# neeek2303/EMOPortraits

Measured on AMD Instinct MI355X. Metric: reenactment frames/sec @512x512, 1-src->N-driver, higher is better.
Workload: dtype f32

## Files before the change

### emoportraits_amd/csrc/conv_igemm_f16x2_p1.h

```cpp
#pragma once
#include "conv_igemm_bf16x3.h"

template <int TR, int TW>
struct ConvCfgP {
  static constexpr int BM = 64, BP = 256, TM = 2, TP = 2, WGP = 4, KC = 32, NPL = 2;
  static constexpr int NQ = TW / 4;
  static constexpr int SUB = ((TR * NQ + 4 + 11) / 16) * 16 + 4;
  static constexpr int CHS = 4 * SUB;
  static constexpr int NG = 4;
  static constexpr int PPL = NG * CHS;
  static constexpr int PBUF = NPL * PPL;
  static constexpr int OFF_P = 0;
  static constexpr int WTILE = NPL * 2 * 2 * BM;
  static constexpr int WTILE_BYTES = WTILE * 16;
  static constexpr int WSTAGE = 2 * WTILE;
  static constexpr int OFF_W = 2 * PBUF;
  static constexpr int OFF_SCT = OFF_W + 2 * WSTAGE;
  static constexpr int SCT = 1024;
  static constexpr int EPI_ROWF = 68;
  static constexpr int EPI_WAVE = 32 * EPI_ROWF;
  static constexpr int OFF_BIAS_F = OFF_SCT * 4 + 2 * SCT;
  static constexpr int OFF_STAT_F = OFF_BIAS_F + BM;
  static constexpr int OFF_BIAS2_F = OFF_STAT_F + 2 * WGP * BM;
  static constexpr int OFF_STAT2_F = OFF_BIAS2_F + BM;
  static constexpr int LDS_BYTES = (OFF_STAT2_F + 2 * WGP * BM) * 4;
  static_assert(TR * TW == BP && TR * NQ == 64, "256 positions = 64 quads: one per lane of the staging wave");
  static_assert(WTILE_BYTES == 8 * 1024, "8 DMA pieces per channel tile and stage");
  static_assert(PBUF * 4 >= WGP * EPI_WAVE, "the epilogue transposes through one patch buffer");
  static_assert(LDS_BYTES <= 160 * 1024, "LDS");
};

template <int TR, int TW>
__global__ __launch_bounds__(256) __attribute__((amdgpu_waves_per_eu(1, 1)))
void conv_igemm_bf16x3_p1_kernel(const ConvArgs a) {
  using Cfg = ConvCfgP<TR, TW>;
  using opx8 = halfx8;
  constexpr int SPLIT = 2, NPL = 2, NPROD = 3;
  constexpr int BM = Cfg::BM, TM = Cfg::TM, TP = Cfg::TP, WGP = Cfg::WGP, KC = Cfg::KC;
  constexpr int NQ = Cfg::NQ, SUB = Cfg::SUB, CHS = Cfg::CHS, PPL = Cfg::PPL, PBUF = Cfg::PBUF;

  extern __shared__ __attribute__((aligned(16))) float smem[];

  EMO_SPLIT_THREAD_IDS()
  const int wp = wave;
  const int p0 = wp * TP * 32;
  float sat_m = 0.0f;

  const int HW = a.H * a.W;
  const long DHW = (long)a.D * HW;
  const bool has_affine = a.scale != nullptr;
  const int epi_mode = __builtin_amdgcn_readfirstlane(a.res == nullptr ? 0 : (a.res_ups ? 2 : 1));
  const float in_scale = a.in_scale;
  constexpr float CLAMP_HI = 65504.0f;
  const float clamp_lo = a.relu_in ? 0.0f : -CLAMP_HI;
  const int nst = a.n_cchunks;
  const int nptiles = a.tiles_x * a.tiles_y * a.tiles_z;
  const int n_cot_all = (a.Cout + BM - 1) / BM;

  const int q_r = lane / NQ, q_c = lane - q_r * NQ;
  int q_slb[4];
#pragma unroll
  for (int i = 0; i < 4; ++i) q_slb[i] = (wave * CHS + i * SUB + lane) * 16;

  floatx16 acc_lo[2][TM][TP], acc_hi[2][TM][TP];

  EMO_SPLIT_ITEM_WALK()
  int it_cotile = 0, it_n = 0, it_ptile = 0, it_x0 = 0, it_y0 = 0, it_z0 = 0;
  unsigned lq_off = 0;
  int lq_z0 = 0;
#define EMO_P1_WPTR(c_, k_) (reinterpret_cast<const char*>(a.wpk) + (long)((c_) * nst + (k_)) * Cfg::WTILE_BYTES)
#define EMO_P1_CURSOR_OF(P_, off_) { off_ = (unsigned)((P_##y0 + q_r) * a.W + P_##x0 + 4 * q_c) * 4u; }

  const int a_off = (half * BM + l32) * 16;
  int b_off[TP];
#pragma unroll
  for (int j = 0; j < TP; ++j) {
    const int p = p0 + j * 32 + l32;
    const int col = p % TW, row = p / TW;
    b_off[j] = (half * CHS + (col & 3) * SUB + row * NQ + (col >> 2)) * 16;
  }
  EMO_SPLIT_LDS_VIEWS()
  opx8 fa_[2][NPL][TM];
  opx8 fb_[2][NPL][TP];
#define EMO_P1_LOAD_A(set_, wb_, h_, ks_)                                                             \
  { _Pragma("unroll") for (int pl = 0; pl < NPL; ++pl) _Pragma("unroll") for (int i = 0; i < TM; ++i) \
      fa_[set_][pl][i] = *reinterpret_cast<const opx8*>(lds_c + a_off + (Cfg::OFF_W + (wb_) * Cfg::WSTAGE + (h_) * Cfg::WTILE + ((pl * 2 + (ks_)) * 2) * BM + i * 32) * 16); }
#define EMO_P1_LOAD_B(pb_, ks_)                                                                       \
  { _Pragma("unroll") for (int pl = 0; pl < NPL; ++pl) _Pragma("unroll") for (int j = 0; j < TP; ++j) \
      fb_[ks_][pl][j] = *reinterpret_cast<const opx8*>(lds_c + b_off[j] + (Cfg::OFF_P + (pb_) * PBUF + pl * PPL + (ks_) * 2 * CHS) * 16); }

  EMO_SPLIT_LDS_TABLES_ADDR()

  floatx4 qv[2][8];
  float q_lo[2], q_hi[2];
  int q_tix[2];
  floatx4 t_sc[2], t_sh[2];
  opx8 cv_h, cv_m;
  emo_intx4 xrs = emo_raw_buffer(a.x);
  EMO_SPLIT_USOFF(8, 0, DHW, 1u)

  int ld_stage;
  unsigned q_vo;
#define EMO_P1_ISSUE_BEGIN(b_)                                                                        \
  EMO_SPLIT_ISSUE_BEGIN([b_], q_vo, ld_stage * KC + wave * 8, cv_, ((unsigned)cs_ * (unsigned)DHW + (unsigned)(lq_z0 * HW)) * 4u)
#define EMO_P1_ISSUE_LOADS(b_) EMO_SPLIT_ISSUE_LOADS(qv[b_], q_vo, 0, 8)
#define EMO_P1_TABLES(b_) EMO_SPLIT_TABLE2(q_tix[b_], t_sc, t_sh)
#define EMO_P1_TOUCH_QUAD(b_) EMO_SPLIT_TOUCH(qv[b_], 8)
#define EMO_P1_CONV_HALF(b_, pb_, i_, hf_)                                                            \
  {                                                                                                   \
    EMO_SPLIT_AFFINE4(t_, qv[b_], 4 * (hf_), i_, t_sc[hf_], t_sh[hf_])                                \
    EMO_SPLIT_RANGE4(t_)                                                                              \
    EMO_SPLIT_F16X2_4(t_, q_lo[b_], q_hi[b_], cv_h, cv_m, 4 * (hf_))                                  \
    if ((hf_) == 1) {                                                                                 \
      char* d_ = lds_w + q_slb[i_] + (Cfg::OFF_P + (pb_) * PBUF) * 16;                                \
      EMO_SPLIT_STORE_PLANES(opx8, d_, cv_h, cv_m)                                                    \
    }                                                                                                 \
  }
#define EMO_P1_DMA_PIECE(ptr0_, ptr1_, wb_, k_)                                                       \
  {                                                                                                   \
    const int j_ = wave + 4 * ((k_) & 1);                                                             \
    emo_dma16_pinned_s((((k_) >> 1) ? (ptr1_) : (ptr0_)) + j_ * 1024, lane16,                         \
                       smem_lds + (unsigned)((Cfg::OFF_W + (wb_) * Cfg::WSTAGE + ((k_) >> 1) * Cfg::WTILE) * 16 + j_ * 1024)); \
  }

  constexpr int PA3[3] = {1, 0, 0}, PB3[3] = {0, 1, 0};
  constexpr int NTE = Cfg::SCT / 256;
  float te_sc[NTE], te_sh[NTE], te_b = 0.0f;

  bool chained_in = false;
  for (int idx8 = blockIdx.x >> 3; idx8 < n_mine; idx8 += l_stride) {
  EMO_SPLIT_DECODE(it_, l_base + idx8, 2 * cot_, )
  int nx_cotile = 0, nx_n = 0, nx_ptile = 0, nx_x0 = 0, nx_y0 = 0, nx_z0 = 0;
  bool chain_out = false;
  unsigned nxq_off = 0;
  if (EMO_S_CHAIN && idx8 + l_stride < n_mine) {
    EMO_SPLIT_DECODE(nx_, l_base + idx8 + l_stride, 2 * cot_, )
    chain_out = nx_n == it_n;
    EMO_P1_CURSOR_OF(nx_, nxq_off)
  }
  (void)nx_ptile;
#pragma unroll
  for (int st_ = 0; st_ < 2; ++st_)
#pragma unroll
    for (int pl = 0; pl < NPL; ++pl) {
#pragma unroll
      for (int i = 0; i < TM; ++i) asm volatile("" : "=v"(fa_[st_][pl][i]));
#pragma unroll
      for (int j = 0; j < TP; ++j) asm volatile("" : "=v"(fb_[st_][pl][j]));
    }
#pragma unroll
  for (int u = 0; u < 8; ++u) asm volatile("" : "=v"(qv[0][u]));
  asm volatile("" : "=v"(cv_h));
  asm volatile("" : "=v"(cv_m));
  if (EMO_S_CHAIN && chained_in) {
    xrs = emo_raw_buffer(a.x + (long)it_n * a.Cin * DHW);
    if (tid < 2 * BM) {
      const int t2_ = tid & (BM - 1);
      smem[(tid < BM ? Cfg::OFF_BIAS_F : Cfg::OFF_BIAS2_F) + (t2_ >> 5) * 32 + (t2_ & 3) * 8 + ((t2_ & 31) >> 2)] = te_b;
    }
    EMO_SPLIT_BARRIER(0);
  } else {
    xrs = emo_raw_buffer(a.x + (long)it_n * a.Cin * DHW);
    EMO_P1_CURSOR_OF(it_, lq_off)
    lq_z0 = it_z0;
#pragma unroll
    for (int k = 0; k < NTE; ++k) {
      const int c = tid + 256 * k;
      const bool real = has_affine && c < a.Cin;
      te_sc[k] = real ? a.scale[(long)it_n * a.Cin + c] : 1.0f;
      te_sh[k] = real ? a.shift[(long)it_n * a.Cin + c] : 0.0f;
    }
    if (tid < 2 * BM && a.bias != nullptr) {
      const int co_ = it_cotile * BM + tid;
      te_b = a.bias[co_ < a.Cout ? co_ : a.Cout - 1];
    }
    {
      const char* const w0_ = EMO_P1_WPTR(it_cotile, 0);
      const char* const w1_ = EMO_P1_WPTR(it_cotile + 1, 0);
#pragma unroll
      for (int k = 0; k < 4; ++k) EMO_P1_DMA_PIECE(w0_, w1_, 0, k)
    }
    ld_stage = 0;
    EMO_P1_ISSUE_BEGIN(0)
    EMO_P1_ISSUE_LOADS(0)
    if (nst > 1) ++ld_stage;
    EMO_P1_ISSUE_BEGIN(1)
    EMO_P1_ISSUE_LOADS(1)
#pragma unroll
    for (int k = 0; k < NTE; ++k) {
      const int c = tid + 256 * k;
      if (c < min(a.Cin, Cfg::SCT)) {
        sct[c] = te_sc[k] * in_scale;
        sct[Cfg::SCT + c] = te_sh[k] * in_scale;
      }
    }
    if (tid < 2 * BM) {
      const int t2_ = tid & (BM - 1);
      smem[(tid < BM ? Cfg::OFF_BIAS_F : Cfg::OFF_BIAS2_F) + (t2_ >> 5) * 32 + (t2_ & 3) * 8 + ((t2_ & 31) >> 2)] = te_b;
    }
    EMO_SPLIT_WAIT(0);
    EMO_P1_TOUCH_QUAD(0)
    EMO_P1_TOUCH_QUAD(1)
    __syncthreads();
    EMO_P1_TABLES(0)
#pragma unroll
    for (int i = 0; i < 4; ++i) {
      EMO_P1_CONV_HALF(0, 0, i, 0)
      EMO_P1_CONV_HALF(0, 0, i, 1)
    }
    EMO_P1_TABLES(1)
    EMO_SPLIT_BARRIER(0);
  }

#pragma unroll
  for (int c = 0; c < 2; ++c)
#pragma unroll
    for (int i = 0; i < TM; ++i)
#pragma unroll
      for (int j = 0; j < TP; ++j)
#pragma unroll
        for (int r = 0; r < 16; ++r) { acc_lo[c][i][j][r] = 0.0f; acc_hi[c][i][j][r] = 0.0f; }
  EMO_P1_LOAD_A(0, 0, 0, 0)
  EMO_P1_LOAD_B(0, 0)
  for (int cg0 = 0; cg0 < nst; cg0 += 2) {
#pragma unroll
    for (int par = 0; par < 2; ++par) {
      const int cg = cg0 + par;
      const bool nx1_ = EMO_S_CHAIN && par == 1 && chain_out && cg + 1 >= nst;
      const int k1_ = nx1_ ? 0 : ((cg + 1) < nst ? cg + 1 : nst - 1);
      const int c1_ = nx1_ ? nx_cotile : it_cotile;
      const char* const dma0 = EMO_P1_WPTR(c1_, k1_);
      const char* const dma1 = EMO_P1_WPTR(c1_ + 1, k1_);
      if (EMO_CONV_SETPRIO) __builtin_amdgcn_s_setprio(1);
#pragma unroll
      for (int gs = 0; gs < 4; ++gs) {
        const int h = gs >> 1, ks = gs & 1;
        const int fcur = gs & 1, fnxt = fcur ^ 1;
        if (gs == 3) { EMO_SPLIT_BARRIER(0); }
        if (gs == 3) EMO_P1_TOUCH_QUAD(par)
        if (gs == 0) {
          const bool sw_ = EMO_S_CHAIN && par == 0 && chain_out && cg + 2 == nst;
          const int tgt_ = (EMO_S_CHAIN && par == 1 && chain_out && cg + 2 > nst) ? 1 : ((cg + 2) < nst ? cg + 2 : nst - 1);
          lq_off = sw_ ? nxq_off : lq_off;
          lq_z0 = sw_ ? nx_z0 : lq_z0;
          ld_stage = sw_ ? 0 : tgt_;
          EMO_P1_ISSUE_BEGIN(par)
        }
        __builtin_amdgcn_sched_barrier(0);
        if (gs < 3) { EMO_P1_LOAD_A(fnxt, par, (gs + 1) >> 1, (gs + 1) & 1) } else { EMO_P1_LOAD_A(fnxt, par ^ 1, 0, 0) }
        if (gs == 0) { EMO_P1_LOAD_B(par, 1) }
        if (gs == 3) { EMO_P1_LOAD_B(par ^ 1, 0) }
        if (gs == 0) EMO_P1_ISSUE_LOADS(par)
        if (gs == 1) {
#pragma unroll
          for (int k = 0; k < 4; ++k) EMO_P1_DMA_PIECE(dma0, dma1, par ^ 1, k)
        }
        if (gs == 0) { EMO_P1_CONV_HALF(par ^ 1, par ^ 1, 0, 0) EMO_P1_CONV_HALF(par ^ 1, par ^ 1, 0, 1) EMO_P1_CONV_HALF(par ^ 1, par ^ 1, 1, 0) }
        if (gs == 1) { EMO_P1_CONV_HALF(par ^ 1, par ^ 1, 1, 1) EMO_P1_CONV_HALF(par ^ 1, par ^ 1, 2, 0) EMO_P1_CONV_HALF(par ^ 1, par ^ 1, 2, 1) }
        if (gs == 2) { EMO_P1_CONV_HALF(par ^ 1, par ^ 1, 3, 0) EMO_P1_CONV_HALF(par ^ 1, par ^ 1, 3, 1) }
        if (gs == 3) { EMO_P1_TABLES(par) }
#pragma unroll
        for (int p = 0; p < NPROD; ++p) {
          const int pa = PA3[p], pb = PB3[p];
#pragma unroll
          for (int i = 0; i < TM; ++i)
#pragma unroll
            for (int j = 0; j < TP; ++j) {
              floatx16& acc_ = (pa == 0 && pb == 0) ? acc_lo[h][i][j] : acc_hi[h][i][j];
              acc_ = __builtin_amdgcn_mfma_f32_32x32x16_f16(fb_[ks][pb][j], fa_[fcur][pa][i], acc_, 0, 0, 0);
            }
        }
        if (EMO_S_PIN) {
#pragma unroll
          for (int k = 0; k < 8; ++k) {
            __builtin_amdgcn_sched_group_barrier(0x008, 1, 0);
            __builtin_amdgcn_sched_group_barrier(0x100, 1, 0);
            __builtin_amdgcn_sched_group_barrier(0x002, 9, 0);
          }
#pragma unroll
          for (int k = 8; k < 4 * NPROD; ++k) {
            __builtin_amdgcn_sched_group_barrier(0x008, 1, 0);
            __builtin_amdgcn_sched_group_barrier(0x002, 10, 0);
            __builtin_amdgcn_sched_group_barrier(0x200, 2, 0);
          }
        }
        __builtin_amdgcn_sched_barrier(0);
      }
      if (EMO_CONV_SETPRIO) __builtin_amdgcn_s_setprio(0);
    }
  }
  {
    const int last_par = (nst - 1) & 1;
    float* const scratch = smem + (Cfg::OFF_P + last_par * PBUF) * 4 + wave * Cfg::EPI_WAVE;
    const int ep_n = it_n, ep_cotile = it_cotile, ep_ptile = it_ptile, ep_x0 = it_x0, ep_y0 = it_y0, ep_z0 = it_z0;
    const bool second = ep_cotile + 1 < n_cot_all;
    EMO_SPLIT_WAIT(0);
    __syncthreads();
    if (EMO_S_CHAIN && chain_out && tid < 2 * BM && a.bias != nullptr) {
      const int co_ = nx_cotile * BM + tid;
      te_b = a.bias[co_ < a.Cout ? co_ : a.Cout - 1];
    }
#define EMO_P1_EPI_FAST(RES_)                                                                         \
    {                                                                                                 \
      floatx4 rv_[8], rvn_[8];                                                                        \
      EMO_SPLIT_EPI_ISSUE(RES_, true, rv_, ep_cotile)                                                 \
      if (second) EMO_SPLIT_EPI_ISSUE(RES_, true, rvn_, ep_cotile + 1)                                \
      EMO_SPLIT_EPI_FINISH(RES_, true, acc_lo[0], acc_hi[0], rv_, Cfg::OFF_BIAS_F, Cfg::OFF_STAT_F, ep_cotile, EMO_SPLIT_NO_STAMPS) \
      if (second) EMO_SPLIT_EPI_FINISH(RES_, true, acc_lo[1], acc_hi[1], rvn_, Cfg::OFF_BIAS2_F, Cfg::OFF_STAT2_F, ep_cotile + 1, EMO_SPLIT_NO_STAMPS) \
    }
    if (epi_mode == 1) EMO_P1_EPI_FAST(1)
    else if (epi_mode == 2) EMO_P1_EPI_FAST(2)
    else EMO_P1_EPI_FAST(0)
#undef EMO_P1_EPI_FAST
  }
  if (a.sat_flag != nullptr && sat_m > 65504.0f) *a.sat_flag = 1;
  __syncthreads();
  if (a.gn_stats != nullptr && tid < 2 * BM && it_cotile * BM + tid < a.Cout) {
    const int c_ = tid & (BM - 1);
    const float* const st_ = smem + (tid < BM ? Cfg::OFF_STAT_F : Cfg::OFF_STAT2_F);
    float mean = 0.0f, m2 = 0.0f;
#pragma unroll
    for (int w = 0; w < WGP; ++w) mean += st_[(w * BM + c_) * 2 + 0];
    mean *= 1.0f / (float)WGP;
#pragma unroll
    for (int w = 0; w < WGP; ++w) {
      const float d = st_[(w * BM + c_) * 2 + 0] - mean;
      m2 += st_[(w * BM + c_) * 2 + 1] + (float)(TP * 32) * d * d;
    }
    float2* dst = reinterpret_cast<float2*>(a.gn_stats) + ((long)it_n * nptiles + it_ptile) * 2 * a.Cout + it_cotile * BM + tid;
    dst[0] = make_float2(mean, 0.5f * m2);
    dst[a.Cout] = make_float2(mean, 0.5f * m2);
  }
  chained_in = chain_out;
  }
#undef EMO_P1_WPTR
#undef EMO_P1_CURSOR_OF
#undef EMO_P1_LOAD_A
#undef EMO_P1_LOAD_B
#undef EMO_P1_ISSUE_BEGIN
#undef EMO_P1_ISSUE_LOADS
#undef EMO_P1_TABLES
#undef EMO_P1_TOUCH_QUAD
#undef EMO_P1_CONV_HALF
#undef EMO_P1_DMA_PIECE
}

template <int TR, int TW>
int conv_f16x2_p1_launch(ConvArgs a, hipStream_t s) {
  using Cfg = ConvCfgP<TR, TW>;
  if (a.KD != 1 || a.ksplit != 1 || a.run_if != nullptr) return EMO_ERR_UNSUPPORTED;
  if (a.Wl % TW || a.Hl % TR || a.Wl != a.W || a.Hl != a.H) return EMO_ERR_UNSUPPORTED;
  if (!conv_input_quads_fit(a, Cfg::SCT) || !conv_straight_epilogue_fits(a, Cfg::BM)) return EMO_ERR_UNSUPPORTED;
  const int cot = a.Cout / Cfg::BM;
  const int pairs = (cot + 1) / 2;
  const long nt = (long)(a.Wl / TW) * (a.Hl / TR) * a.Dl;
  if (nt > 0x7fffffffL || a.N > 65535 || nt * pairs * a.N > 0x7fffffffL) return EMO_ERR_UNSUPPORTED;
  auto kern = conv_igemm_bf16x3_p1_kernel<TR, TW>;
  const int rc = emo_raise_dynamic_lds(kern);
  if (rc != EMO_OK) return rc;
  a.tiles_x = a.Wl / TW;
  a.tiles_y = a.Hl / TR;
  a.tiles_z = a.Dl;
  a.n_cchunks = (a.Cin + Cfg::KC - 1) / Cfg::KC;
  if (a.n_cchunks & 1) return EMO_ERR_UNSUPPORTED;
  a.stages_per_split = a.n_cchunks;
  a.partial = nullptr;
  a.cot0 = 0;
  a.n_cotiles = pairs;
  a.n_work = (int)(nt * pairs * a.N);
  const int ncu = emo_cu_count();
  const int grid = a.n_work > ncu ? ncu : a.n_work;
  return emo_launch(kern, dim3((unsigned)grid), dim3(256), (size_t)Cfg::LDS_BYTES, s, a);
}
```

Measured before the change: 417.1.

## Deepen input prefetch pipeline to three stages and hoist affine transform

The input quad loads are now issued one stage further ahead: prologue issues stage 2, the main loop targets cg+3, and the two qv register buffers alternate. The per-channel affine (scale/shift FMA) is split into a separate step that runs once per stage into a cvq buffer, so the conversion halves no longer recompute it. Barriers now wait with a nonzero outstanding-load count so more loads can stay in flight, and DMA of weights moves to gs==0. The aim is to hide global-load latency behind the MFMA loop. In exchange it costs extra VGPRs for cvq and the second qv set, and chaining is restricted to nst>=4. Ablation switches are added but default to off.

```diff
diff --git a/emoportraits_amd/csrc/conv_igemm_f16x2_p1.h b/emoportraits_amd/csrc/conv_igemm_f16x2_p1.h
--- a/emoportraits_amd/csrc/conv_igemm_f16x2_p1.h
+++ b/emoportraits_amd/csrc/conv_igemm_f16x2_p1.h
@@ -1,5 +1,8 @@
 #pragma once
 #include "conv_igemm_bf16x3.h"
+#ifndef EMO_P1_ABLATE
+#define EMO_P1_ABLATE 0
+#endif
 
 template <int TR, int TW>
 struct ConvCfgP {
@@ -68,7 +71,7 @@
   int it_cotile = 0, it_n = 0, it_ptile = 0, it_x0 = 0, it_y0 = 0, it_z0 = 0;
   unsigned lq_off = 0;
   int lq_z0 = 0;
-#define EMO_P1_WPTR(c_, k_) (reinterpret_cast<const char*>(a.wpk) + (long)((c_) * nst + (k_)) * Cfg::WTILE_BYTES)
+#define EMO_P1_WPTR(c_, k_) (reinterpret_cast<const char*>(a.wpk) + (EMO_P1_ABLATE == 2 ? 0l : (long)((c_) * nst + (k_)) * Cfg::WTILE_BYTES))
 #define EMO_P1_CURSOR_OF(P_, off_) { off_ = (unsigned)((P_##y0 + q_r) * a.W + P_##x0 + 4 * q_c) * 4u; }
 
   const int a_off = (half * BM + l32) * 16;
@@ -92,25 +95,33 @@
   EMO_SPLIT_LDS_TABLES_ADDR()
 
   floatx4 qv[2][8];
-  float q_lo[2], q_hi[2];
+  floatx4 cvq[8];
+  float q_lo[2], q_hi[2], c_lo, c_hi;
   int q_tix[2];
   floatx4 t_sc[2], t_sh[2];
   opx8 cv_h, cv_m;
   emo_intx4 xrs = emo_raw_buffer(a.x);
-  EMO_SPLIT_USOFF(8, 0, DHW, 1u)
+  EMO_SPLIT_USOFF(8, 0, DHW, (EMO_P1_ABLATE == 3 ? 0u : 1u))
 
   int ld_stage;
   unsigned q_vo;
 #define EMO_P1_ISSUE_BEGIN(b_)                                                                        \
-  EMO_SPLIT_ISSUE_BEGIN([b_], q_vo, ld_stage * KC + wave * 8, cv_, ((unsigned)cs_ * (unsigned)DHW + (unsigned)(lq_z0 * HW)) * 4u)
+  EMO_SPLIT_ISSUE_BEGIN([b_], q_vo, ld_stage * KC + wave * 8, cv_, ((EMO_P1_ABLATE == 3 ? 0u : (unsigned)cs_ * (unsigned)DHW) + (unsigned)(lq_z0 * HW)) * 4u)
 #define EMO_P1_ISSUE_LOADS(b_) EMO_SPLIT_ISSUE_LOADS(qv[b_], q_vo, 0, 8)
 #define EMO_P1_TABLES(b_) EMO_SPLIT_TABLE2(q_tix[b_], t_sc, t_sh)
 #define EMO_P1_TOUCH_QUAD(b_) EMO_SPLIT_TOUCH(qv[b_], 8)
-#define EMO_P1_CONV_HALF(b_, pb_, i_, hf_)                                                            \
+#define EMO_P1_AFFINE(b_)                                                                             \
   {                                                                                                   \
-    EMO_SPLIT_AFFINE4(t_, qv[b_], 4 * (hf_), i_, t_sc[hf_], t_sh[hf_])                                \
+    _Pragma("unroll") for (int u = 0; u < 8; ++u) _Pragma("unroll") for (int i = 0; i < 4; ++i)       \
+      cvq[u][i] = __fmaf_rn(qv[b_][u][i], t_sc[u >> 2][u & 3], t_sh[u >> 2][u & 3]);                  \
+    c_lo = q_lo[b_]; c_hi = q_hi[b_];                                                                 \
+  }
+#define EMO_P1_CONV_HALF(pb_, i_, hf_)                                                                \
+  {                                                                                                   \
+    float t_[4];                                                                                      \
+    _Pragma("unroll") for (int k = 0; k < 4; ++k) t_[k] = cvq[4 * (hf_) + k][i_];                     \
     EMO_SPLIT_RANGE4(t_)                                                                              \
-    EMO_SPLIT_F16X2_4(t_, q_lo[b_], q_hi[b_], cv_h, cv_m, 4 * (hf_))                                  \
+    EMO_SPLIT_F16X2_4(t_, c_lo, c_hi, cv_h, cv_m, 4 * (hf_))                                          \
     if ((hf_) == 1) {                                                                                 \
       char* d_ = lds_w + q_slb[i_] + (Cfg::OFF_P + (pb_) * PBUF) * 16;                                \
       EMO_SPLIT_STORE_PLANES(opx8, d_, cv_h, cv_m)                                                    \
@@ -135,7 +146,7 @@
   unsigned nxq_off = 0;
   if (EMO_S_CHAIN && idx8 + l_stride < n_mine) {
     EMO_SPLIT_DECODE(nx_, l_base + idx8 + l_stride, 2 * cot_, )
-    chain_out = nx_n == it_n;
+    chain_out = nx_n == it_n && nst >= 4;
     EMO_P1_CURSOR_OF(nx_, nxq_off)
   }
   (void)nx_ptile;
@@ -149,7 +160,7 @@
       for (int j = 0; j < TP; ++j) asm volatile("" : "=v"(fb_[st_][pl][j]));
     }
 #pragma unroll
-  for (int u = 0; u < 8; ++u) asm volatile("" : "=v"(qv[0][u]));
+  for (int u = 0; u < 8; ++u) asm volatile("" : "=v"(qv[1][u]));
   asm volatile("" : "=v"(cv_h));
   asm volatile("" : "=v"(cv_m));
   if (EMO_S_CHAIN && chained_in) {
@@ -160,6 +171,11 @@
     }
     EMO_SPLIT_BARRIER(0);
   } else {
+#pragma unroll
+    for (int u = 0; u < 8; ++u) {
+      asm volatile("" : "=v"(qv[0][u]));
+      asm volatile("" : "=v"(cvq[u]));
+    }
     xrs = emo_raw_buffer(a.x + (long)it_n * a.Cin * DHW);
     EMO_P1_CURSOR_OF(it_, lq_off)
     lq_z0 = it_z0;
@@ -203,13 +219,18 @@
     EMO_P1_TOUCH_QUAD(1)
     __syncthreads();
     EMO_P1_TABLES(0)
+    EMO_P1_AFFINE(0)
+    ld_stage = nst > 2 ? 2 : nst - 1;
+    EMO_P1_ISSUE_BEGIN(0)
+    EMO_P1_ISSUE_LOADS(0)
 #pragma unroll
     for (int i = 0; i < 4; ++i) {
-      EMO_P1_CONV_HALF(0, 0, i, 0)
-      EMO_P1_CONV_HALF(0, 0, i, 1)
+      EMO_P1_CONV_HALF(0, i, 0)
+      EMO_P1_CONV_HALF(0, i, 1)
     }
     EMO_P1_TABLES(1)
-    EMO_SPLIT_BARRIER(0);
+    EMO_P1_AFFINE(1)
+    EMO_SPLIT_BARRIER(8);
   }
 
 #pragma unroll
@@ -222,7 +243,8 @@
         for (int r = 0; r < 16; ++r) { acc_lo[c][i][j][r] = 0.0f; acc_hi[c][i][j][r] = 0.0f; }
   EMO_P1_LOAD_A(0, 0, 0, 0)
   EMO_P1_LOAD_B(0, 0)
-  for (int cg0 = 0; cg0 < nst; cg0 += 2) {
+  int cg0 = 0;
+  do {
 #pragma unroll
     for (int par = 0; par < 2; ++par) {
       const int cg = cg0 + par;
@@ -236,29 +258,32 @@
       for (int gs = 0; gs < 4; ++gs) {
         const int h = gs >> 1, ks = gs & 1;
         const int fcur = gs & 1, fnxt = fcur ^ 1;
-        if (gs == 3) { EMO_SPLIT_BARRIER(0); }
+        if (gs == 3) { if (EMO_P1_ABLATE == 7) EMO_SPLIT_WAIT(8); else EMO_SPLIT_BARRIER(EMO_P1_ABLATE == 1 ? 63 : 8); }
         if (gs == 3) EMO_P1_TOUCH_QUAD(par)
         if (gs == 0) {
-          const bool sw_ = EMO_S_CHAIN && par == 0 && chain_out && cg + 2 == nst;
-          const int tgt_ = (EMO_S_CHAIN && par == 1 && chain_out && cg + 2 > nst) ? 1 : ((cg + 2) < nst ? cg + 2 : nst - 1);
+          const bool sw_ = EMO_S_CHAIN && par == 1 && chain_out && cg + 3 == nst;
+          const int tgt_ = (EMO_S_CHAIN && chain_out && cg + 3 > nst) ? 1 + par : ((cg + 3) < nst ? cg + 3 : nst - 1);
           lq_off = sw_ ? nxq_off : lq_off;
           lq_z0 = sw_ ? nx_z0 : lq_z0;
           ld_stage = sw_ ? 0 : tgt_;
-          EMO_P1_ISSUE_BEGIN(par)
+          EMO_P1_ISSUE_BEGIN(par ^ 1)
         }
         __builtin_amdgcn_sched_barrier(0);
         if (gs < 3) { EMO_P1_LOAD_A(fnxt, par, (gs + 1) >> 1, (gs + 1) & 1) } else { EMO_P1_LOAD_A(fnxt, par ^ 1, 0, 0) }
         if (gs == 0) { EMO_P1_LOAD_B(par, 1) }
         if (gs == 3) { EMO_P1_LOAD_B(par ^ 1, 0) }
-        if (gs == 0) EMO_P1_ISSUE_LOADS(par)
-        if (gs == 1) {
-#pragma unroll
-          for (int k = 0; k < 4; ++k) EMO_P1_DMA_PIECE(dma0, dma1, par ^ 1, k)
+        if (gs == 0) {
+#pragma unroll
+          for (int k = 0; k < (EMO_P1_ABLATE != 4 ? 4 : 0); ++k) EMO_P1_DMA_PIECE(dma0, dma1, par ^ 1, k)
+          if (EMO_P1_ABLATE != 5) EMO_P1_ISSUE_LOADS(par ^ 1)
         }
-        if (gs == 0) { EMO_P1_CONV_HALF(par ^ 1, par ^ 1, 0, 0) EMO_P1_CONV_HALF(par ^ 1, par ^ 1, 0, 1) EMO_P1_CONV_HALF(par ^ 1, par ^ 1, 1, 0) }
-        if (gs == 1) { EMO_P1_CONV_HALF(par ^ 1, par ^ 1, 1, 1) EMO_P1_CONV_HALF(par ^ 1, par ^ 1, 2, 0) EMO_P1_CONV_HALF(par ^ 1, par ^ 1, 2, 1) }
-        if (gs == 2) { EMO_P1_CONV_HALF(par ^ 1, par ^ 1, 3, 0) EMO_P1_CONV_HALF(par ^ 1, par ^ 1, 3, 1) }
-        if (gs == 3) { EMO_P1_TABLES(par) }
+        if (EMO_P1_ABLATE != 6) {
+        if (gs == 0) { EMO_P1_CONV_HALF(par ^ 1, 0, 0) EMO_P1_CONV_HALF(par ^ 1, 0, 1) EMO_P1_CONV_HALF(par ^ 1, 1, 0) }
+        if (gs == 1) { EMO_P1_CONV_HALF(par ^ 1, 1, 1) EMO_P1_CONV_HALF(par ^ 1, 2, 0) EMO_P1_CONV_HALF(par ^ 1, 2, 1) }
+        if (gs == 2) { EMO_P1_CONV_HALF(par ^ 1, 3, 0) EMO_P1_CONV_HALF(par ^ 1, 3, 1) }
+        }
+        if (gs == 2) { EMO_P1_TABLES(par) }
+        if (gs == 3) { EMO_P1_AFFINE(par) }
 #pragma unroll
         for (int p = 0; p < NPROD; ++p) {
           const int pa = PA3[p], pb = PB3[p];
@@ -288,13 +313,15 @@
       }
       if (EMO_CONV_SETPRIO) __builtin_amdgcn_s_setprio(0);
     }
-  }
+    cg0 += 2;
+  } while (cg0 < nst);
   {
     const int last_par = (nst - 1) & 1;
     float* const scratch = smem + (Cfg::OFF_P + last_par * PBUF) * 4 + wave * Cfg::EPI_WAVE;
     const int ep_n = it_n, ep_cotile = it_cotile, ep_ptile = it_ptile, ep_x0 = it_x0, ep_y0 = it_y0, ep_z0 = it_z0;
     const bool second = ep_cotile + 1 < n_cot_all;
     EMO_SPLIT_WAIT(0);
+    EMO_P1_TOUCH_QUAD(0)
     __syncthreads();
     if (EMO_S_CHAIN && chain_out && tid < 2 * BM && a.bias != nullptr) {
       const int co_ = nx_cotile * BM + tid;
@@ -341,6 +368,7 @@
 #undef EMO_P1_ISSUE_LOADS
 #undef EMO_P1_TABLES
 #undef EMO_P1_TOUCH_QUAD
+#undef EMO_P1_AFFINE
 #undef EMO_P1_CONV_HALF
 #undef EMO_P1_DMA_PIECE
 }
```

After: 417.2, median of 3. About the same (+0.0%).
